# haoxiangsnr/Wave-U-Net-for-Speech-Enhancement

Hardware: AMD Instinct MI355X
Metric: 16384-sample frames/sec fwd+bwd, 12-level Wave-U-Net (higher is better)
Workload: dtype f32 (levels >= 16 samples: 3 x f16 MFMA on hi/lo fp16 halves, fp32 accumulate; the rest f32 MFMA); 1 GPU; unet_basic 12-level, 16384-sample frames, batch=64 per GPU, fp32, training-mode forward + smooth_l1 + backward + fused HIP Adam step (BASELINE.json configs[2]; configs[3] when n_gpus>1); global_batch=64, frame=16384, parallelism=dp1

## Files before the change

wave-u-net-for-speech-enhancement_amd/csrc/wunet_elementwise.h:

```cpp
#pragma once
#include "wunet_dev.h"

struct PackDesc {
    const float* w;
    float* dst;
    int Cout, Cin, taps;
    int M;
    int CP;
    int mtiles;
    int transposed;
};

#define WUNET_MAX_CONV_LAYERS 34
struct PackTable { PackDesc d[WUNET_MAX_CONV_LAYERS]; };

static __global__ __launch_bounds__(WUNET_THREADS) void pack_weights_kernel(PackTable tab)
{
    const PackDesc& d = tab.d[blockIdx.y];
    const int total = d.mtiles * d.CP * d.taps * 16;
    const int kc = d.transposed ? d.Cout : d.Cin;
    for (int idx = blockIdx.x * WUNET_THREADS + threadIdx.x; idx < total; idx += gridDim.x * WUNET_THREADS) {
        const int i = idx & 15;
        int r = idx >> 4;
        const int t = r % d.taps; r /= d.taps;
        const int c = r % d.CP;
        const int mt = r / d.CP;
        const int m = mt * 16 + i;
        float v = 0.0f;
        if (m < d.M && c < kc) {
            v = d.transposed ? d.w[((size_t)c * d.Cin + m) * d.taps + (d.taps - 1 - t)]
                             : d.w[((size_t)m * d.Cin + c) * d.taps + t];
        }
        d.dst[idx] = v;
    }
}

template <int N>
__device__ __forceinline__ void block_sum(double (&a)[N], double* red)
{
// ... 1213 lines not shown
```

wave-u-net-for-speech-enhancement_amd/csrc/wunet_forward.cpp:

```cpp
#include "wunet_host.h"
#include "wunet_elementwise.h"
#include "wunet_tiny.h"
#include "wunet_h3_elem.h"

using namespace wunet_host;

namespace {
struct FwdMode {
    bool training, save;
    const unsigned char* frozen;
    bool is_frozen(int i) const { return frozen && i >= 0 && frozen[i] != 0; }
};

bool skip_handoff(const wunet_ctx* c, int d, const FwdMode& m)
{
    if (!m.training || d <= c->n || d >= c->NL) return false;
    const LayerPlan& dl = c->ly[d];
    return dl.skip_from > 0 && !dl.h3u_train && !m.is_frozen(dl.src0) && !m.is_frozen(dl.src1);
}
bool evop_handoff(const wunet_ctx* c, int p, const FwdMode& m) { return !m.training && p >= 0 && p < c->NL && c->ly[p].evop; }

enum { OP_NONE = 0, OP_IN_CONV, OP_BY_PRODUCER, OP_PREP_H3, OP_SCALAR, OP_DECIM, OP_UPCAT };
enum { CV_FIRST = 0, CV_H3U, CV_H3, CV_TINY, CV_FP32 };
enum { BOUND_NONE = 0, BOUND_EPILOGUE, BOUND_REDUCE, BOUND_ACT_MAX };
// ... 78 lines not shown
};
struct FwdSides { wunet_ctx::Side* fwd = nullptr; wunet_ctx::Side* bwd = nullptr; };

int fork_side(wunet_ctx::Side* side, hipStream_t st)
{
    if (hipEventRecord(side->ev_fork, st) != hipSuccess || hipStreamWaitEvent(side->stream, side->ev_fork, 0) != hipSuccess)
        return fail(WUNET_E_RUNTIME, "fork onto the side stream failed");
    return WUNET_OK;
}

int pack_fp32(const FwdCall& k, hipStream_t pst)
{
    wunet_ctx* c = k.c;
    PackTable tab{};
    int nd = 0;
    for (int i = 0; i < c->NL; ++i) {
        const LayerPlan& l = c->ly[i];
        if (l.h3f || l.first) continue;
        PackDesc& d = tab.d[nd++];
        d.w = k.params[4 * i]; d.dst = k.ws + c->wpkf_off + l.f_wpk;
        d.Cout = l.cout; d.Cin = l.cin; d.taps = l.taps; d.M = l.cout; d.CP = l.f.cp; d.mtiles = l.f.mtiles_p; d.transposed = 0;
    }
    if (nd > 0) {
        WUNET_LAUNCH(pack_weights_kernel, dim3(pack_gx(), nd), dim3(WUNET_THREADS), 0, pst, tab);
        WUNET_CHECK_LAUNCH();
    }
    return WUNET_OK;
}

int pack_split(const FwdCall& k, hipStream_t pst)
{
    wunet_ctx* c = k.c; float* ws = k.ws;
    const bool training = k.m.training;
    {
        ScaleTable T{};
        bool any = false;
        for (int i = 0; i < c->NL; ++i) {
            const LayerPlan& l = c->ly[i];
            ScaleDesc& d = T.d[i];
            d.w = (l.h3f || l.h3d) ? k.params[4 * i] : nullptr; d.wn = (unsigned)((size_t)l.cout * l.cin * l.taps);
            d.gamma = k.params[4 * i + 2]; d.beta = k.params[4 * i + 3]; d.C = l.cout;
            d.sqrtn = sqrtf((float)((double)c->B * l.Lt));
            d.frozen = k.m.is_frozen(i) ? 1 : 0;
            d.zp0 = l.h3f ? ws + l.xzp : nullptr;
            d.zp1 = (l.h3d && training && k.m.save) ? ws + l.gzp : nullptr;
            any = any || l.h3f;
        }
        T.wmax = ws + c->wmax_off; T.slots = x_scale_slot(c, ws, 0); T.training = training ? 1 : 0;
        if (any) {
            WUNET_LAUNCH(h3_scales_kernel, dim3(WUNET_WMAX_PARTS, c->NL), dim3(WUNET_THREADS), 0, pst, T);
            WUNET_CHECK_LAUNCH();
        }
    }
    PackH3Table tab{};
    int nd = 0;
    wunet_half* wh = reinterpret_cast<wunet_half*>(ws + c->h3_wf_hi);
    wunet_half* wl = reinterpret_cast<wunet_half*>(ws + c->h3_wf_lo);
    for (int i = 0; i < c->NL; ++i) {
        const LayerPlan& l = c->ly[i];
        if (!l.h3f) continue;
        PackH3Desc& d = tab.d[nd++];
        d.w = k.params[4 * i]; d.hi = wh + l.h3f_wpk; d.lo = wl + l.h3f_wpk;
        d.Cout = l.cout; d.Cin = l.cin; d.taps = l.taps; d.rows = l.cout; d.kch = l.cin; d.mtiles = l.hf.mtp; d.nch = l.hf.nch; d.transposed = 0;
        d.ntt = (training ? l.h3u_train : l.h3u) ? 0 : l.hf.ntt; d.nfull = ((l.cin + 7) / 8) / 4; d.ns = h3_stage_count(l.cin, l.taps, d.ntt);
        d.wmax = ws + c->wmax_off + (size_t)WUNET_WMAX_PARTS * i; d.wsc = w_scale_slot(c, ws, i);
        d.bf = c->bf;
    }
    if (nd > 0) {
        WUNET_LAUNCH(pack_h3_kernel, dim3(pack_gx(), nd), dim3(WUNET_THREADS), 0, pst, tab);
        WUNET_CHECK_LAUNCH();
    }
    if (!training) {
        RowL1Table rt{};
        int nr = 0;
        for (int i = 0; i < c->NL; ++i) {
            const LayerPlan& l = c->ly[i];
            if (!l.evop) continue;
            RowL1Desc& d = rt.d[nr++];
            d.w = k.params[4 * i]; d.dst = ws + l.wl1; d.rows = l.cout; d.rowlen = l.cin * l.taps;
        }
        if (nr > 0) {
            WUNET_LAUNCH(w_rowl1_kernel, dim3(8, nr), dim3(WUNET_THREADS), 0, pst, rt);
            WUNET_CHECK_LAUNCH();
        }
    }
    return WUNET_OK;
}

int forward_packs(const FwdCall& k, bool packs_valid, void* workspace, FwdSides& sides)
{
    wunet_ctx* c = k.c; float* ws = k.ws; const hipStream_t st = k.st;
    const bool training = k.m.training;
// ... 284 lines not shown
```

wave-u-net-for-speech-enhancement_amd/csrc/wunet_h3_elem.h:

```cpp
#pragma once
#include "wunet_elementwise.h"
#include "wunet_h3.h"

#define WUNET_SLOT_FLOATS 8
#define WUNET_WMAX_PARTS 64
struct ScaleDesc {
    const float* w; unsigned wn;
    const float* gamma; const float* beta; int C;
    float sqrtn;
    int frozen;
    float* zp0; float* zp1;
};
struct ScaleTable { ScaleDesc d[WUNET_MAX_CONV_LAYERS]; float* wmax; float* slots; int training; };

static __global__ __launch_bounds__(WUNET_THREADS) void h3_scales_kernel(ScaleTable T)
{
    __shared__ float red[WUNET_THREADS];
    const ScaleDesc& d = T.d[blockIdx.y];
    const int tid = threadIdx.x;
    if (d.w) {
        float m = 0.0f;
        for (unsigned i = blockIdx.x * WUNET_THREADS + tid; i < d.wn; i += gridDim.x * WUNET_THREADS) m = fmaxf(m, fabsf(d.w[i]));
        red[tid] = m;
        __syncthreads();
        for (int s = WUNET_THREADS / 2; s > 0; s >>= 1) {
            if (tid < s) red[tid] = fmaxf(red[tid], red[tid + s]);
            __syncthreads();
        }
        if (tid == 0) T.wmax[blockIdx.y * WUNET_WMAX_PARTS + blockIdx.x] = red[0];
        __syncthreads();
    }
    if (blockIdx.x == 0) {
        float m = 0.0f;
        if (T.training && !d.frozen)
            for (int c = tid; c < d.C; c += WUNET_THREADS) m = fmaxf(m, fabsf(d.gamma[c]) * d.sqrtn + fabsf(d.beta[c]));
        red[tid] = m;
        __syncthreads();
        for (int s = WUNET_THREADS / 2; s > 0; s >>= 1) {
            if (tid < s) red[tid] = fmaxf(red[tid], red[tid + s]);
            __syncthreads();
        }
        if (tid == 0) T.slots[blockIdx.y * WUNET_SLOT_FLOATS + 4] = red[0];
        if (tid < 4) {
            if (d.zp0) d.zp0[tid] = 0.0f;
            if (d.zp1) d.zp1[tid] = 0.0f;
        }
    }
}

struct RowL1Desc { const float* w; float* dst; int rows, rowlen; };
struct RowL1Table { RowL1Desc d[WUNET_MAX_CONV_LAYERS]; };
static __global__ __launch_bounds__(WUNET_THREADS) void w_rowl1_kernel(RowL1Table T)
{
    __shared__ float red[WUNET_WAVES];
    const RowL1Desc& d = T.d[blockIdx.y];
    for (int r = blockIdx.x; r < d.rows; r += gridDim.x) {
        const float* wr = d.w + (size_t)r * d.rowlen;
        float m = 0.0f;
        for (int i = threadIdx.x; i < d.rowlen; i += WUNET_THREADS) m += fabsf(wr[i]);
#pragma unroll
        for (int k = 1; k < 64; k <<= 1) m += wunet_shfl_xor(m, k);
        __syncthreads();
        if ((threadIdx.x & 63) == 0) red[threadIdx.x >> 6] = m;
        __syncthreads();
        if (threadIdx.x == 0) d.dst[r] = (red[0] + red[1]) + (red[2] + red[3]);
    }
}

static __global__ __launch_bounds__(WUNET_THREADS) void h3_slots_clear_kernel(ScaleTable T, int nl)
{
// ... 440 lines not shown
                    wunet_put_half(l, e, d);
                }
                wunet_sth8(A.sh + (srow * (size_t)(2 * A.L) + (size_t)q) * 8, h);
                if (!A.bf) wunet_sth8(A.sl + (srow * (size_t)(2 * A.L) + (size_t)q) * 8, l);
            }
        }
    }
}

struct PackH3Desc {
    const float* w;
    wunet_half* hi;
    wunet_half* lo;
    int Cout, Cin, taps;
    int rows, kch;
    int mtiles, nch;
    int transposed;
    const float* wmax;
    float* wsc;
    int bf;
    int ntt;
    int nfull, ns;
};
struct PackH3Table { PackH3Desc d[WUNET_MAX_CONV_LAYERS]; };

static __global__ __launch_bounds__(WUNET_THREADS) void pack_h3_kernel(PackH3Table tab)
{
    const PackH3Desc& d = tab.d[blockIdx.y];
    const int ntg = d.taps / 5, ns = d.ntt ? d.ns : d.nch * ntg, nfs = d.ntt ? d.nfull * ntg : ns;
    const int total = d.mtiles * ns * 5 * 512;
    __shared__ float wsc_sh[2];
    if (threadIdx.x < 64) {
        float m = threadIdx.x < WUNET_WMAX_PARTS ? d.wmax[threadIdx.x] : 0.0f;
#pragma unroll
        for (int k = 1; k < 64; k <<= 1) m = fmaxf(m, wunet_shfl_xor(m, k));
        if (threadIdx.x == 0) {
            float s_, i_;
            wunet_pow2_scale(m, s_, i_);
            wsc_sh[0] = s_; wsc_sh[1] = i_;
            if (blockIdx.x == 0 && d.wsc) { d.wsc[0] = s_; d.wsc[1] = i_; }
        }
    }
    __syncthreads();
    const float wscale = wsc_sh[0];
    for (int idx = blockIdx.x * WUNET_THREADS + threadIdx.x; idx < total; idx += gridDim.x * WUNET_THREADS) {
        const int e = idx & 7, i = (idx >> 3) & 15, q = (idx >> 7) & 3;
        int r = idx >> 9;
        const int slot = r % 5; r /= 5;
        const int stg = r % ns, mt = r / ns;
        const int row = mt * 16 + i;
        int k, t;
        if (stg < nfs) { k = (stg / ntg) * 32 + q * 8 + e; t = (stg % ntg) * 5 + slot; }
        else { k = d.nfull * 32 + (stg - nfs) * 8 + e; t = slot < d.ntt ? q * d.ntt + slot : d.taps; }
        float v = 0.0f;
        if (row < d.rows && k < d.kch && t < d.taps)
            v = d.transposed ? d.w[((size_t)k * d.Cin + row) * d.taps + (d.taps - 1 - t)] : d.w[((size_t)row * d.Cin + k) * d.taps + t];
        wunet_half a, b;
        wunet_split_rt(d.bf, wscale * v, a, b);
        d.hi[idx] = a;
        if (!d.bf) d.lo[idx] = b;
    }
}
```

wave-u-net-for-speech-enhancement_amd/csrc/wunet_host.h:

```cpp
#pragma once
#include <cstdarg>
#include <cmath>
#include <cstdio>
#include <cstdlib>
#include <cstring>
#include <map>
#include <mutex>
#include <string>
#include <vector>

#include "wunet_kernels.h"
#include "wunet_h3.h"
#include "wunet_h3u.h"
#include "wunet_launch.h"
#include "wunet_hip.h"

namespace wunet_host {

int fail(int code, const char* fmt, ...);
const char* last_error_text();

#define WUNET_CHECK_LAUNCH()                                                                   \
    do {                                                                                       \
        hipError_t e_ = hipGetLastError();                                                     \
// ... 8 lines not shown

inline int ilog2(long long v) { int r = 0; while ((1LL << r) < v) ++r; return r; }
inline bool is_pow2(long long v) { return v > 0 && (v & (v - 1)) == 0; }
inline size_t align64(size_t v) { return (v + 63) & ~(size_t)63; }
inline int round_up(int v, int m) { return (v + m - 1) / m * m; }
inline unsigned capped_blocks(size_t n, size_t per_block, size_t cap) { const size_t b = (n + per_block - 1) / per_block; return (unsigned)(b < cap ? b : cap); }
inline int kc_of(int taps) { return wunet_lds::conv_mfma(taps, 1).kc; }

struct ConvCfg { int mrep, nrep, mtiles_p, mblocks, cp, grid_x, ksplit, kcps; };
ConvCfg plan_conv(int B, int L, int rows, int kch, int taps);
ConvArgs make_conv_args(const float* x, int kch, const float* wpk, const float* bias, float* out, float* stats,
                        int B, int rows, int L, int taps, const ConvCfg& c, size_t split_stride);
int launch_conv(int taps, const ConvArgs& a, const ConvCfg& c, hipStream_t st);

struct WgradCfg { int mrep, nw, xit, wsplit, mblocks, nblocks, ksplit, cps, rows; };
WgradCfg plan_wgrad(int B, int L, int cin, int cout, int taps);
WgradArgs make_wgrad_args(const float* x, const float* g, float* part, int B, int Cin, int Cout, int L, int taps, int cps);
int launch_wgrad_any(int taps, const WgradArgs& a, const WgradCfg& w, hipStream_t st);

enum { LK_RAW = 0, LK_DECIM = 1, LK_UPCAT = 2 };

struct PlanSwitches {
    const char *order_f, *order_d, *order_w;
    bool no_split, old_split, ktail_off, no_skip_fuse, no_evop, no_e0, no_enc_gz, pa_swap_off, upt_off, wgrad_xcd_off;
    int sps, h3u_eval, h3u_train, a_cap;
};
PlanSwitches read_plan_switches();

struct H3ConvPlan { int mrep, mtp, nch, sps, ksplit, ntiles, ntt; };
H3ConvPlan plan_h3_conv(int B, int L, int rows, int kch, int taps, bool transposed, int bf, const PlanSwitches& sw);
struct H3WgradPlan { int mrep, mblocks, nblocks, ksplit, cps, tp, xcd, dma, db; };
H3WgradPlan plan_h3_wgrad(int B, int L, int cin, int cout, int taps, int bf, const PlanSwitches& sw);

struct LayerGeom {
    int cin, cout, taps, L, logL, kind;
    int Lt;
    int src0, src1;
    int c0;
};
struct LayerDecisions {
    ConvCfg f;
    ConvCfg d;
    WgradCfg w;
    int f_rows;
    int a_split;
    size_t f_wpk, d_wpk;
    size_t z, a, s, mean, rstd, xin, g, dx, k1, k2, k3;
// ... 16 lines not shown
struct LayerPlan : LayerGeom, LayerDecisions {};

int h3_stage_count(int kch, int taps, int ntt);
size_t h3w_part_stride(const LayerGeom& g, const H3WgradPlan& w);
int wgrad_blocks_per_cu(const WgradCfg& w, int L, int taps);
int h3w_blocks_per_cu(int taps, int mrep, int L);
bool up_pairs_regular(int Lin);
unsigned pack_gx();

}

struct wunet_ctx {
    int n, ci, B, T, NL;
    int Tt = 0;
    bool padded = false;
    size_t pad_in = 0, pad_out = 0, pad_gout = 0;
    std::vector<wunet_host::LayerPlan> ly;
    size_t stats_off, wpkf_off, spart_off, fwd_floats;
    size_t bmax_off, bound_off;
    size_t bpart_off, wgpart_off, wpkb_off, gh_off, hpart_off, hpart2_off, e0part_off, total_floats;
    int e0 = 1;
    int enc_gz = 1;
    int pa_swap = 1;
    int head_blocks;
    int h3 = 0;
    int bf = 0;
    std::vector<unsigned char> frozen;
    bool any_frozen = false;
    size_t h3_wf_hi, h3_wf_lo, h3_wb_hi, h3_wb_lo, h3_slot;
    size_t fslot_off, wmax_off;
    size_t h3_wf_halfs, h3_wb_halfs;
    struct Side {
        hipStream_t stream = nullptr; hipEvent_t ev_fork = nullptr, ev_join = nullptr, ev_pack = nullptr, ev_fpack = nullptr, ev_fpack2 = nullptr;
        const void* packed_ws = nullptr;
    };
    std::map<int, Side> side;
    std::mutex side_lock;
};

namespace wunet_host {

void layout_workspace(wunet_ctx* c);
int launch_split(const float* x, wunet_half* hi, wunet_half* lo, const float* sc, const float* xb0, const float* xb1, float* xsc,
                 int B, int C, int L, hipStream_t st, int bf = 0);
float* x_scale_slot(const wunet_ctx* c, float* ws, int layer);
float* w_scale_slot(const wunet_ctx* c, float* ws, int layer);
// ... 25 lines not shown
```

wave-u-net-for-speech-enhancement_amd/csrc/wunet_launchers.cpp:

```cpp
#include "wunet_host.h"
#include "wunet_elementwise.h"
#include "wunet_h3_elem.h"

namespace wunet_host {

static int lds_refused(const char* kernel, size_t smem)
{
    return fail(WUNET_E_ARG, "%s: %zu bytes of dynamic LDS requested, its layout needs %zu", kernel, smem, wunet_lds_needed);
}

ConvArgs make_conv_args(const float* x, int kch, const float* wpk, const float* bias, float* out, float* stats,
                        int B, int rows, int L, int taps, const ConvCfg& c, size_t split_stride)
{
    ConvArgs a{};
    a.x = x; a.wpk = wpk; a.bias = bias; a.out = out; a.stats = stats;
    a.B = B; a.Cin = kch; a.Cout = rows; a.CinP = c.cp; a.L = L; a.logL = ilog2(L);
    const int tn = 64 * c.nrep;
    a.seg = L < tn ? L : tn;
    a.seg_shift = ilog2(a.seg);
    a.segw = a.seg + 16;
    const int rowlen = wunet_lds::staged_row(L, tn);
    a.rowp = wunet_lds::conv_mfma_rowp(L, c.nrep);
    a.r4 = rowlen / 4;
    a.sw4 = a.segw / 4;
// ... 184 lines not shown
        WgradH3Args a{};
        fill(a);
        rc = wunet_launch_wgrad_h3(a, l.taps, w.mrep, nseg, tp, grid, smem, st, bf != 0);
    }
    prof_end(st);
    if (rc == WUNET_LAUNCH_E_LDS) return lds_refused(pname, smem);
    if (rc != 0) return fail(WUNET_E_ARG, "no wgrad_h3 kernel for taps=%d mrep=%d (rc %d)", l.taps, w.mrep, rc);
    return 0;
}

int launch_backward_packs(wunet_ctx* c, const float* const* params, float* ws, hipStream_t st)
{
    const int NL = c->NL;
    PackTable tab{};
    int nd = 0;
    for (int i = 1; i < NL; ++i) {
        const LayerPlan& l = c->ly[i];
        if (l.h3d) continue;
        PackDesc& d = tab.d[nd++];
        d.w = params[4 * i]; d.dst = ws + c->wpkb_off + l.d_wpk;
        d.Cout = l.cout; d.Cin = l.cin; d.taps = l.taps; d.M = l.cin; d.CP = l.d.cp; d.mtiles = l.d.mtiles_p; d.transposed = 1;
    }
    if (nd > 0) {
        WUNET_LAUNCH(pack_weights_kernel, dim3(pack_gx(), nd), dim3(WUNET_THREADS), 0, st, tab);
        WUNET_CHECK_LAUNCH();
    }
    if (c->h3) {
        PackH3Table t3{};
        int n3 = 0;
        wunet_half* wh = reinterpret_cast<wunet_half*>(ws + c->h3_wb_hi);
        wunet_half* wl = reinterpret_cast<wunet_half*>(ws + c->h3_wb_lo);
        for (int i = 1; i < NL; ++i) {
            const LayerPlan& l = c->ly[i];
            if (!l.h3d) continue;
            PackH3Desc& d = t3.d[n3++];
            d.w = params[4 * i]; d.hi = wh + l.h3d_wpk; d.lo = wl + l.h3d_wpk;
            d.Cout = l.cout; d.Cin = l.cin; d.taps = l.taps; d.rows = l.cin; d.kch = l.cout; d.mtiles = l.hd.mtp; d.nch = l.hd.nch; d.transposed = 1;
            d.ntt = l.hd.ntt; d.nfull = ((l.cout + 7) / 8) / 4; d.ns = h3_stage_count(l.cout, l.taps, l.hd.ntt);
            d.wmax = ws + c->wmax_off + (size_t)WUNET_WMAX_PARTS * i;
            d.wsc = l.h3f ? nullptr : w_scale_slot(c, ws, i);
            d.bf = c->bf;
        }
        if (n3 > 0) {
            WUNET_LAUNCH(pack_h3_kernel, dim3(pack_gx(), n3), dim3(WUNET_THREADS), 0, st, t3);
            WUNET_CHECK_LAUNCH();
        }
    }
    return 0;
}

bool side_stream_off()
{
    static const bool off = getenv("WUNET_NO_SIDE_STREAM") != nullptr;
    return off;
}

wunet_ctx::Side* side_for_current_device(wunet_ctx* c)
{
    int dev = 0;
    if (hipGetDevice(&dev) != hipSuccess) { fail(WUNET_E_RUNTIME, "hipGetDevice failed"); return nullptr; }
    std::lock_guard<std::mutex> g(c->side_lock);
    auto it = c->side.find(dev);
    if (it != c->side.end()) return &it->second;
    wunet_ctx::Side sd;
    const unsigned evf = hipEventDisableTiming | (unsigned)hipEventDisableSystemFence;
    if (hipStreamCreateWithFlags(&sd.stream, hipStreamNonBlocking) != hipSuccess ||
        hipEventCreateWithFlags(&sd.ev_fork, evf) != hipSuccess ||
// ... 12 lines not shown
```

wave-u-net-for-speech-enhancement_amd/csrc/wunet_ops.cpp:

```cpp
#include "wunet_host.h"
#include "wunet_elementwise.h"
#include "wunet_h3_elem.h"
#include "wunet_loss_rows.h"
#include "wunet_stft.h"
#include "wunet_stoi.h"
#include "wunet_estoi.h"
#include "wunet_mix.h"
#include "wunet_reverb.h"

using namespace wunet_host;

extern "C" {

size_t wunet_loss_scratch_bytes(void) { return 256 * sizeof(double); }

int wunet_loss_forward(int kind, const float* clean, const float* enhanced, size_t n, float* loss_out, void* scratch, void* stream)
{
    if (kind < 0 || kind > 2 || !clean || !enhanced || !loss_out || !scratch || n == 0) return fail(WUNET_E_ARG, "bad loss argument");
    hipStream_t st = (hipStream_t)stream;
    const unsigned blocks = capped_blocks(n, WUNET_THREADS * 8, 256);
    WUNET_LAUNCH(loss_partial_kernel, dim3(blocks), dim3(WUNET_THREADS), 0, st, kind, clean, enhanced, n, (double*)scratch);
    WUNET_CHECK_LAUNCH();
    WUNET_LAUNCH(loss_final_kernel, dim3(1), dim3(WUNET_THREADS), 0, st, (const double*)scratch, (int)blocks, n, loss_out);
    WUNET_CHECK_LAUNCH();
// ... 744 lines not shown
    prof_end(st);
    WUNET_CHECK_LAUNCH();
    return WUNET_OK;
}

static int op_check(int B, int Cin, int Cout, int L, int K)
{
    if (K != 5 && K != 15) return fail(WUNET_E_ARG, "K must be 5 or 15");
    if (B < 1 || Cin < 1 || Cout < 1 || !is_pow2(L) || L < 4) return fail(WUNET_E_ARG, "bad op shape (L must be a power of two >= 4)");
    return 0;
}

static int op_conv_common(const float* x, const float* w, const float* bias, float* out, int B, int kch, int rows,
                          int Cout, int Cin, int L, int K, int transposed, hipStream_t st)
{
    const ConvCfg cfg = plan_conv(B, L, rows, kch, K);
    float *wpk = nullptr, *part = nullptr;
    if (hipMalloc((void**)&wpk, (size_t)cfg.mtiles_p * cfg.cp * K * 16 * sizeof(float)) != hipSuccess) return fail(WUNET_E_RUNTIME, "hipMalloc");
    const size_t nout = (size_t)B * rows * L;
    if (cfg.ksplit > 1 && hipMalloc((void**)&part, (size_t)cfg.ksplit * nout * sizeof(float)) != hipSuccess) return fail(WUNET_E_RUNTIME, "hipMalloc");
    PackTable tab{};
    PackDesc& d = tab.d[0];
    d.w = w; d.dst = wpk; d.Cout = Cout; d.Cin = Cin; d.taps = K; d.M = rows; d.CP = cfg.cp; d.mtiles = cfg.mtiles_p; d.transposed = transposed;
    WUNET_LAUNCH(pack_weights_kernel, dim3(64, 1), dim3(WUNET_THREADS), 0, st, tab);
    const bool split = cfg.ksplit > 1;
    const ConvArgs a = make_conv_args(x, kch, wpk, split ? nullptr : bias, split ? part : out, nullptr, B, rows, L, K, cfg, nout);
    int rc = launch_conv(K, a, cfg, st);
    if (!rc && split) {
        WUNET_LAUNCH(split_sum_kernel, dim3(capped_blocks(nout, WUNET_THREADS, 2048)), dim3(WUNET_THREADS), 0, st, (const float*)part, cfg.ksplit, nout, out,
                     bias, rows, ilog2(L));
    }
    hipStreamSynchronize(st);
    hipFree(wpk);
    if (part) hipFree(part);
    if (rc) return rc;
    WUNET_CHECK_LAUNCH();
    return WUNET_OK;
}

int wunet_op_conv1d(const float* x, const float* w, const float* bias, float* z, int B, int Cin, int Cout, int L, int K, void* stream)
{
    if (op_check(B, Cin, Cout, L, K)) return WUNET_E_ARG;
    return op_conv_common(x, w, bias, z, B, Cin, Cout, Cout, Cin, L, K, 0, (hipStream_t)stream);
}

int wunet_op_conv1d_dgrad(const float* gz, const float* w, float* dx, int B, int Cin, int Cout, int L, int K, void* stream)
{
// ... 60 lines not shown
}

int op_conv_split_common(const float* x, const float* w, const float* bias, float* out, int B, int kch, int rows, int Cout, int Cin,
                         int L, int K, int transposed, int bf, hipStream_t st)
{
    const H3ConvPlan p = plan_h3_conv(B, L, rows, kch, K, transposed != 0, bf, read_plan_switches());
    SplitBuf xs;
    DevBuf wpk, misc, part;
    const size_t wh_halfs = (size_t)p.mtp * p.nch * K * 512, nout = (size_t)B * rows * L;
    if (!wpk.alloc(wh_halfs * 4) || !misc.alloc((16 + WUNET_WMAX_PARTS + 2 * (size_t)kch) * sizeof(float)) ||
        (p.ksplit > 1 && !part.alloc((size_t)p.ksplit * nout * sizeof(float))))
        return fail(WUNET_E_RUNTIME, "hipMalloc");
    float* xslot = misc.f(), *wslot = misc.f() + 8, *wmax = misc.f() + 16, *oz = misc.f() + 16 + WUNET_WMAX_PARTS;
    WUNET_LAUNCH(fill_kernel, dim3(4), dim3(WUNET_THREADS), 0, st, oz, (size_t)kch, 1.0f);
    WUNET_LAUNCH(fill_kernel, dim3(4), dim3(WUNET_THREADS), 0, st, oz + kch, (size_t)kch, 0.0f);
    wunet_half* const whp = wpk.h();
    wunet_half* const wlp = wpk.h() + wh_halfs;
    int rc = op_split_operand(x, B, kch, L, xs, xslot, oz, oz + kch, bf, st);
    if (rc) return rc;
    {
        ScaleTable T{};
        T.d[0].w = w; T.d[0].wn = (unsigned)((size_t)Cout * Cin * K); T.d[0].gamma = oz; T.d[0].beta = oz; T.d[0].C = 1; T.d[0].sqrtn = 0.0f;
        T.wmax = wmax; T.slots = wslot; T.training = 0;
        WUNET_LAUNCH(h3_scales_kernel, dim3(WUNET_WMAX_PARTS, 1), dim3(WUNET_THREADS), 0, st, T);
        PackH3Table tab{};
        PackH3Desc& d = tab.d[0];
        d.w = w; d.hi = whp; d.lo = wlp; d.Cout = Cout; d.Cin = Cin; d.taps = K; d.rows = rows; d.kch = kch; d.mtiles = p.mtp; d.nch = p.nch;
        d.ntt = p.ntt; d.nfull = ((kch + 7) / 8) / 4; d.ns = h3_stage_count(kch, K, p.ntt);
        d.transposed = transposed; d.wmax = wmax; d.wsc = wslot + 2; d.bf = bf;
        WUNET_LAUNCH(pack_h3_kernel, dim3(64, 1), dim3(WUNET_THREADS), 0, st, tab);
    }
    const bool split = p.ksplit > 1;
    ConvH3Launch h{};
    h.taps = K; h.mrep = p.mrep; h.mtiles_p = p.mtp; h.sps = p.sps; h.nch = p.nch; h.ntt = p.ntt;
    h.B = B; h.rows = rows; h.kch = kch; h.L = L; h.bf = bf;
    h.xh = xs.h(); h.xl = xs.l(); h.zpad = xs.zpad(); h.wh = whp; h.wl = wlp;
    h.bias = split ? nullptr : bias; h.sc = xslot; h.sc2 = wslot + 2; h.out = split ? part.f() : out;
    rc = launch_conv_h3(h, st);
    if (!rc && split) {
        const unsigned blocks = capped_blocks(nout, WUNET_THREADS, 2048);
        const float* partp = part.f();
        const int ks = p.ksplit;
        char pname[48];
        snprintf(pname, sizeof pname, "split_sum_kernel<%d>", ks);
        prof_begin(st, pname, 0.0, 4.0 * (ks + 1.0) * nout);
        WUNET_LAUNCH(split_sum_kernel, dim3(blocks), dim3(WUNET_THREADS), 0, st, partp, ks, nout, out, bias, rows, ilog2(L));
        prof_end(st);
    }
    hipStreamSynchronize(st);
    if (rc) return rc;
    WUNET_CHECK_LAUNCH();
    return WUNET_OK;
}
// ... 69 lines not shown
```

wave-u-net-for-speech-enhancement_amd/csrc/wunet_plan.cpp:

```cpp
#include <algorithm>
#include "wunet_host.h"
#include "wunet_h3_elem.h"

namespace wunet_host {

namespace { thread_local std::string g_err; }

int fail(int code, const char* fmt, ...)
{
    char buf[512];
    va_list ap;
    va_start(ap, fmt);
    vsnprintf(buf, sizeof buf, fmt, ap);
    va_end(ap);
    g_err = buf;
    return code;
}

const char* last_error_text() { return g_err.c_str(); }

namespace {
struct ProfRec { std::string name; double flops; double bytes; hipEvent_t e0, e1; };
std::vector<ProfRec> g_prof;
}
// ... 163 lines not shown
    w.rows = w.ksplit * (w.wsplit ? 4 : 1);
    return w;
}
unsigned pack_gx() { return 512; }

PlanSwitches read_plan_switches()
{
    const auto is_zero = [](const char* name) { const char* e = getenv(name); return e != nullptr && atoi(e) == 0; };
    PlanSwitches sw{};
    sw.order_f = getenv("WUNET_H3_ORDER"); sw.order_d = getenv("WUNET_H3D_ORDER"); sw.order_w = getenv("WUNET_H3W_ORDER");
    sw.no_split = getenv("WUNET_H3_NOSPLIT") != nullptr; sw.old_split = getenv("WUNET_H3_OLDSPLIT") != nullptr;
    if (const char* e = getenv("WUNET_H3_SPS")) sw.sps = atoi(e);
    sw.ktail_off = is_zero("WUNET_H3_KTAIL");
    sw.h3u_eval = 512; sw.h3u_train = 2048;
    if (const char* e = getenv("WUNET_H3U")) {
        int a = 0, b = 0;
        const int got = sscanf(e, "%d,%d", &a, &b);
        if (got == 2) { sw.h3u_eval = a; sw.h3u_train = b; }
        else if (got == 1) sw.h3u_eval = sw.h3u_train = a;
    }
    sw.no_skip_fuse = getenv("WUNET_NO_SKIP_FUSE") != nullptr; sw.no_evop = getenv("WUNET_NO_EVOP") != nullptr; sw.no_e0 = getenv("WUNET_NO_E0") != nullptr;
    sw.no_enc_gz = getenv("WUNET_NO_ENC_GZ") != nullptr; sw.pa_swap_off = is_zero("WUNET_PA_SWAP");
    sw.upt_off = is_zero("WUNET_UPT"); sw.wgrad_xcd_off = is_zero("WUNET_WGRAD_XCD");
    sw.a_cap = getenv("WUNET_A_CAP") ? atoi(getenv("WUNET_A_CAP")) : 128;
    return sw;
}

int pick_mrep_h3(int mtiles, const char* ord)
{
    int best = 2, best_pad = 1 << 30;
    for (const char* p = ord; *p; ++p) {
        const int m = *p - '0';
        const int pad = round_up(mtiles, m) - mtiles;
        if (pad < best_pad) { best_pad = pad; best = m; }
    }
    return best;
}

const char* h3_order(int taps, int L, int ntiles, int mtiles)
{
    return (taps == 5 && L >= 256 && (long long)ntiles * ((mtiles + 3) / 4) >= 512) ? "432" : "32";
}

size_t h3w_part_stride(const LayerGeom& g, const H3WgradPlan& w)
{
    const int tw = g.taps == 15 ? 8 : 5;
// ... 131 lines not shown
        l.h3x = l.h3w;
        if (l.h3f) {
            l.hf = plan_h3_conv(B, l.L, l.cout, l.cin, l.taps, false, c->bf, sw);
            l.f.ksplit = l.hf.ksplit;
            l.f.grid_x = l.hf.ntiles;
        }
        if (l.h3d) {
            l.hd = plan_h3_conv(B, l.L, l.cin, l.cout, l.taps, true, c->bf, sw);
            l.d.ksplit = l.hd.ksplit;
        }
        if (l.h3w) l.hw = plan_h3_wgrad(B, l.L, l.cin, l.cout, l.taps, c->bf, sw);
        if (l.first) { l.f.ksplit = 1; l.f.grid_x = (int)(((long long)B * l.L + 1023) / 1024); }
        const bool can = h3u_can_run(c, l);
        l.h3u = (can && sw.h3u_eval > 0 && l.L >= sw.h3u_eval) ? 1 : 0;
        l.h3u_train = (can && sw.h3u_train > 0 && l.L >= sw.h3u_train) ? 1 : 0;
        l.f_rows = l.h3f ? l.f.grid_x : l.f.grid_x * WUNET_WAVES;
        const long long sp = posn / 4096;
        const int a_cap = sw.a_cap < 1 ? 1 : (sw.a_cap > 256 ? 256 : sw.a_cap);
        l.a_split = (int)(sp < 1 ? 1 : (sp > a_cap ? a_cap : sp));
    }
    const long long hb = ((long long)B * c->T) / 2048;
    c->head_blocks = (int)(hb < 1 ? 1 : (hb > 1024 ? 1024 : hb));
    c->e0 = sw.no_e0 ? 0 : 1;
    c->enc_gz = sw.no_enc_gz ? 0 : 1;
    c->pa_swap = sw.pa_swap_off ? 0 : 1;
}

static bool skip_planned(const LayerPlan& e, const LayerPlan& d) { return e.kind == LK_DECIM && d.kind == LK_UPCAT && e.h3x && d.h3x && d.src1 == e.src0 && d.c0 % 8 == 0; }
static bool evop_planned(const wunet_ctx* c, const LayerPlan& p, const LayerPlan& q, int pi)
{
    return p.h3f && !p.first && p.taps == 15 && p.L >= 256 && p.f.ksplit == 1 && p.hf.mrep <= 4 && q.kind == LK_DECIM && q.src0 == pi && q.h3f && q.h3x &&
           !c->bf && !c->padded;
}
static bool upt_planned(const wunet_ctx* c, const LayerPlan& q, const LayerPlan& p)
{
    return q.kind == LK_UPCAT && q.h3d && q.L >= 256 && q.d.ksplit == 1 && !(q.c0 & 3) && !(q.cin & 3) && q.c0 == p.cout && !c->bf && !c->padded &&
           p.h3d && p.L >= 128 && up_pairs_regular(q.L / 2);
}
static void plan_handoffs(wunet_ctx* c, const PlanSwitches& sw)
{
    for (int i = 1; i <= c->n && !sw.no_skip_fuse; ++i) {
        LayerPlan& d = c->ly[2 * c->n - i + 1];
        if (skip_planned(c->ly[i], d)) d.skip_from = i;
    }
    for (int i = 1; i + 1 <= c->n && !sw.no_evop; ++i)
        if (evop_planned(c, c->ly[i], c->ly[i + 1], i)) c->ly[i].evop = 1;
// ... 204 lines not shown
```

Before: 12770 frames/s.

## Pack weights through LDS tiles with coalesced vector loads instead of strided gathers

Replaces the per-element gather weight packing kernels (fp32 and hi/lo fp16 split) with tiled kernels. Each block loads a 16-row by 32-channel weight tile into shared memory using aligned float4 loads, then writes packed output with vector stores, and the grid is flattened across layers through a prefix table. The weight abs-max scale kernel is also vectorised with float4 loads and wave shuffles. The old gather kernels remain available behind WUNET_PACK_GATHER. Weight packing runs every step, so this targets the per-step pre-processing cost, at the expense of more complex code and handling for misalignment and tails.

```diff
diff --git a/wave-u-net-for-speech-enhancement_amd/csrc/wunet_elementwise.h b/wave-u-net-for-speech-enhancement_amd/csrc/wunet_elementwise.h
--- a/wave-u-net-for-speech-enhancement_amd/csrc/wunet_elementwise.h
+++ b/wave-u-net-for-speech-enhancement_amd/csrc/wunet_elementwise.h
@@ -12,9 +12,119 @@
 };
 
 #define WUNET_MAX_CONV_LAYERS 34
-struct PackTable { PackDesc d[WUNET_MAX_CONV_LAYERS]; };
-
+struct PackTable { PackDesc d[WUNET_MAX_CONV_LAYERS]; int first[WUNET_MAX_CONV_LAYERS + 1]; };
+
+template <int TAPS, bool TR, int PAD>
+struct WTileShape {
+    static constexpr int RUNS = TR ? 32 : 16, LEN = (TR ? 16 : 32) * TAPS, STRIDE = LEN + PAD;
+    static constexpr int NPR = LEN / 4 + 1;
+    static constexpr int PPL = (NPR + 63) / 64;
+    static constexpr int NLD = RUNS / WUNET_WAVES * PPL;
+    static __device__ __forceinline__ int at(int i, int kk, int t) { return TR ? kk * STRIDE + i * TAPS + (TAPS - 1 - t) : i * STRIDE + kk * TAPS + t; }
+};
+#define WUNET_WTILE_FLOATS (32 * (16 * 15 + 2))
+struct WTileSrc { unsigned start, step; int nruns, nlen; };
+__device__ __forceinline__ int wunet_clampi(int v, int hi) { return v < 0 ? 0 : (v > hi ? hi : v); }
+__device__ __forceinline__ WTileSrc wunet_wtile_src(bool transposed, int Cin, int taps, int row0, int nrows, int k0, int nk)
+{
+    WTileSrc T;
+    T.step = (unsigned)(Cin * taps);
+    if (transposed) { T.start = ((unsigned)k0 * Cin + row0) * taps; T.nruns = nk; T.nlen = nrows * taps; }
+    else { T.start = ((unsigned)row0 * Cin + k0) * taps; T.nruns = nrows; T.nlen = nk * taps; }
+    return T;
+}
+template <class S>
+__device__ __forceinline__ void wunet_wtile_load(float* tile, const float* w, const WTileSrc& T)
+{
+    float ev = 0.0f;
+    int eat = -1;
+    {
+        const int r = (int)threadIdx.x >> 3, k = (int)threadIdx.x & 7;
+        if (r < T.nruns) {
+            const float* a = w + (T.start + (unsigned)r * T.step);
+            const int mis = (int)(((size_t)a >> 2) & 3), g = k < 4 ? 0 : (T.nlen + mis) / 4, p = 4 * g - mis, pos = p + (k & 3);
+            const bool whole = p >= 0 && p + 4 <= T.nlen;
+            if ((k < 4 || g > 0) && !whole && pos >= 0 && pos < T.nlen) { ev = a[pos]; eat = r * S::STRIDE + pos; }
+        }
+    }
+    const int wave = wunet_uniform((int)threadIdx.x >> 6), lane = (int)threadIdx.x & 63;
+    wunet_f4 v[S::NLD];
+    bool ld[S::NLD];
+#pragma unroll
+    for (int k = 0; k < S::NLD; ++k) {
+        const int r = wave + WUNET_WAVES * (k / S::PPL), g = lane + 64 * (k % S::PPL);
+        ld[k] = false;
+        if (r < T.nruns && g < S::NPR) {
+            const float* a = w + (T.start + (unsigned)r * T.step);
+            const int p = 4 * g - (int)(((size_t)a >> 2) & 3);
+            if (p >= 0 && p + 4 <= T.nlen) { v[k] = wunet_ld4(a + p); ld[k] = true; }
+        }
+    }
+    if (eat >= 0) tile[eat] = ev;
+#pragma unroll
+    for (int k = 0; k < S::NLD; ++k) {
+        const int r = wave + WUNET_WAVES * (k / S::PPL), g = lane + 64 * (k % S::PPL);
+        if (g >= S::NPR) continue;
+        const bool in = r < T.nruns;
+        const int mis = in ? (int)(((size_t)(w + (T.start + (unsigned)r * T.step)) >> 2) & 3) : 0, p = 4 * g - mis;
+        if (ld[k]) {
+#pragma unroll
+            for (int e = 0; e < 4; ++e) tile[r * S::STRIDE + p + e] = v[k][e];
+        } else {
+            const int ne = in ? T.nlen : 0;
+#pragma unroll
+            for (int e = 0; e < 4; ++e) {
+                const int q = p + e;
+                if (q >= ne && q < S::LEN) tile[r * S::STRIDE + q] = 0.0f;
+            }
+        }
+    }
+}
+
+template <int TAPS, bool TR>
+__device__ __forceinline__ void pack_weights_tile(const PackDesc& d, int mt, int ch, float* tile)
+{
+    typedef WTileShape<TAPS, TR, 2> S;
+    const int kc = TR ? d.Cout : d.Cin;
+    wunet_wtile_load<S>(tile, d.w, wunet_wtile_src(TR, d.Cin, TAPS, mt * 16, wunet_clampi(d.M - mt * 16, 16), ch * 32, wunet_clampi(kc - ch * 32, 32)));
+    __syncthreads();
+    const int np = wunet_clampi(d.CP - ch * 32, 32) * TAPS * 4;
+    float* out = d.dst + ((size_t)mt * d.CP + ch * 32) * TAPS * 16;
+    for (int p = threadIdx.x; p < np; p += WUNET_THREADS) {
+        const int i4 = p & 3, ct = p >> 2, cc = ct / TAPS, t = ct - cc * TAPS;
+        wunet_f4 v;
+#pragma unroll
+        for (int j = 0; j < 4; ++j) v[j] = tile[S::at(i4 * 4 + j, cc, t)];
+        wunet_st4(out + 4 * (size_t)p, v);
+    }
+}
 static __global__ __launch_bounds__(WUNET_THREADS) void pack_weights_kernel(PackTable tab)
+{
+    __shared__ float tile[WUNET_WTILE_FLOATS];
+    int li = 0;
+    while ((int)blockIdx.x >= tab.first[li + 1]) ++li;
+    const PackDesc& d = tab.d[li];
+    const int nch = (d.CP + 31) / 32, u = (int)blockIdx.x - tab.first[li], mt = u / nch, ch = u - mt * nch;
+    if (d.taps == 15) {
+        if (d.transposed) pack_weights_tile<15, true>(d, mt, ch, tile);
+        else pack_weights_tile<15, false>(d, mt, ch, tile);
+    } else {
+        if (d.transposed) pack_weights_tile<5, true>(d, mt, ch, tile);
+        else pack_weights_tile<5, false>(d, mt, ch, tile);
+    }
+}
+
+inline unsigned pack_table_blocks(PackTable& tab, int nd)
+{
+    int n = 0;
+    for (int i = 0; i <= WUNET_MAX_CONV_LAYERS; ++i) {
+        tab.first[i] = n;
+        if (i < nd) n += tab.d[i].mtiles * ((tab.d[i].CP + 31) / 32);
+    }
+    return (unsigned)n;
+}
+
+static __global__ __launch_bounds__(WUNET_THREADS) void pack_weights_gather_kernel(PackTable tab)
 {
     const PackDesc& d = tab.d[blockIdx.y];
     const int total = d.mtiles * d.CP * d.taps * 16;
diff --git a/wave-u-net-for-speech-enhancement_amd/csrc/wunet_forward.cpp b/wave-u-net-for-speech-enhancement_amd/csrc/wunet_forward.cpp
--- a/wave-u-net-for-speech-enhancement_amd/csrc/wunet_forward.cpp
+++ b/wave-u-net-for-speech-enhancement_amd/csrc/wunet_forward.cpp
@@ -124,7 +124,9 @@
         d.Cout = l.cout; d.Cin = l.cin; d.taps = l.taps; d.M = l.cout; d.CP = l.f.cp; d.mtiles = l.f.mtiles_p; d.transposed = 0;
     }
     if (nd > 0) {
-        WUNET_LAUNCH(pack_weights_kernel, dim3(pack_gx(), nd), dim3(WUNET_THREADS), 0, pst, tab);
+        const unsigned tiles = pack_table_blocks(tab, nd);
+        if (c->pack_gather) WUNET_LAUNCH(pack_weights_gather_kernel, dim3(pack_gx(), nd), dim3(WUNET_THREADS), 0, pst, tab);
+        else WUNET_LAUNCH(pack_weights_kernel, dim3(tiles), dim3(WUNET_THREADS), 0, pst, tab);
         WUNET_CHECK_LAUNCH();
     }
     return WUNET_OK;
@@ -150,7 +152,8 @@
         }
         T.wmax = ws + c->wmax_off; T.slots = x_scale_slot(c, ws, 0); T.training = training ? 1 : 0;
         if (any) {
-            WUNET_LAUNCH(h3_scales_kernel, dim3(WUNET_WMAX_PARTS, c->NL), dim3(WUNET_THREADS), 0, pst, T);
+            if (c->pack_gather) WUNET_LAUNCH(h3_scales_gather_kernel, dim3(WUNET_WMAX_PARTS, c->NL), dim3(WUNET_THREADS), 0, pst, T);
+            else WUNET_LAUNCH(h3_scales_kernel, dim3(WUNET_WMAX_PARTS, c->NL), dim3(WUNET_THREADS), 0, pst, T);
             WUNET_CHECK_LAUNCH();
         }
     }
@@ -169,7 +172,9 @@
         d.bf = c->bf;
     }
     if (nd > 0) {
-        WUNET_LAUNCH(pack_h3_kernel, dim3(pack_gx(), nd), dim3(WUNET_THREADS), 0, pst, tab);
+        const unsigned tiles = pack_table_blocks(tab, nd);
+        if (c->pack_gather) WUNET_LAUNCH(pack_h3_gather_kernel, dim3(pack_gx(), nd), dim3(WUNET_THREADS), 0, pst, tab);
+        else WUNET_LAUNCH(pack_h3_kernel, dim3(tiles), dim3(WUNET_THREADS), 0, pst, tab);
         WUNET_CHECK_LAUNCH();
     }
     if (!training) {
diff --git a/wave-u-net-for-speech-enhancement_amd/csrc/wunet_h3_elem.h b/wave-u-net-for-speech-enhancement_amd/csrc/wunet_h3_elem.h
--- a/wave-u-net-for-speech-enhancement_amd/csrc/wunet_h3_elem.h
+++ b/wave-u-net-for-speech-enhancement_amd/csrc/wunet_h3_elem.h
@@ -13,7 +13,72 @@
 };
 struct ScaleTable { ScaleDesc d[WUNET_MAX_CONV_LAYERS]; float* wmax; float* slots; int training; };
 
+__device__ __forceinline__ void h3_scales_bound(const ScaleTable& T, const ScaleDesc& d, float* red)
+{
+    const int tid = threadIdx.x;
+    {
+        float m = 0.0f;
+        if (T.training && !d.frozen)
+            for (int c = tid; c < d.C; c += WUNET_THREADS) m = fmaxf(m, fabsf(d.gamma[c]) * d.sqrtn + fabsf(d.beta[c]));
+        red[tid] = m;
+        __syncthreads();
+        for (int s = WUNET_THREADS / 2; s > 0; s >>= 1) {
+            if (tid < s) red[tid] = fmaxf(red[tid], red[tid + s]);
+            __syncthreads();
+        }
+        if (tid == 0) T.slots[blockIdx.y * WUNET_SLOT_FLOATS + 4] = red[0];
+        if (tid < 4) {
+            if (d.zp0) d.zp0[tid] = 0.0f;
+            if (d.zp1) d.zp1[tid] = 0.0f;
+        }
+    }
+}
+
+__device__ __forceinline__ float wunet_absmax4(float m, wunet_f4 v)
+{
+    return fmaxf(fmaxf(m, fabsf(v[0])), fmaxf(fmaxf(fabsf(v[1]), fabsf(v[2])), fabsf(v[3])));
+}
+
 static __global__ __launch_bounds__(WUNET_THREADS) void h3_scales_kernel(ScaleTable T)
+{
+    __shared__ float red[WUNET_THREADS];
+    const ScaleDesc& d = T.d[blockIdx.y];
+    const int tid = threadIdx.x;
+    if (d.w) {
+        const unsigned mis = (unsigned)(((size_t)d.w >> 2) & 3), h4 = (4u - mis) & 3u, head = h4 < d.wn ? h4 : d.wn;
+        const unsigned n4 = (d.wn - head) / 4, tail = d.wn - head - 4 * n4, stride = gridDim.x * WUNET_THREADS;
+        const float* body = d.w + head;
+        float m0 = 0.0f, m1 = 0.0f, m2 = 0.0f, m3 = 0.0f;
+        unsigned i = blockIdx.x * WUNET_THREADS + tid;
+        for (; i + 7 * stride < n4; i += 8 * stride) {
+            wunet_f4 v[8];
+#pragma unroll
+            for (int k = 0; k < 8; ++k) v[k] = wunet_ld4(body + 4 * (size_t)(i + k * stride));
+            m0 = wunet_absmax4(wunet_absmax4(m0, v[0]), v[4]); m1 = wunet_absmax4(wunet_absmax4(m1, v[1]), v[5]);
+            m2 = wunet_absmax4(wunet_absmax4(m2, v[2]), v[6]); m3 = wunet_absmax4(wunet_absmax4(m3, v[3]), v[7]);
+        }
+        for (; i + 3 * stride < n4; i += 4 * stride) {
+            const wunet_f4 v0 = wunet_ld4(body + 4 * (size_t)i), v1 = wunet_ld4(body + 4 * (size_t)(i + stride));
+            const wunet_f4 v2 = wunet_ld4(body + 4 * (size_t)(i + 2 * stride)), v3 = wunet_ld4(body + 4 * (size_t)(i + 3 * stride));
+            m0 = wunet_absmax4(m0, v0); m1 = wunet_absmax4(m1, v1); m2 = wunet_absmax4(m2, v2); m3 = wunet_absmax4(m3, v3);
+        }
+        for (; i < n4; i += stride) m0 = wunet_absmax4(m0, wunet_ld4(body + 4 * (size_t)i));
+        if (blockIdx.x == 0) {
+            if ((unsigned)tid < head) m1 = fmaxf(m1, fabsf(d.w[tid]));
+            if ((unsigned)tid < tail) m2 = fmaxf(m2, fabsf(body[4 * (size_t)n4 + tid]));
+        }
+        float m = fmaxf(fmaxf(m0, m1), fmaxf(m2, m3));
+#pragma unroll
+        for (int k = 1; k < 64; k <<= 1) m = fmaxf(m, wunet_shfl_xor(m, k));
+        if ((tid & 63) == 0) red[tid >> 6] = m;
+        __syncthreads();
+        if (tid == 0) T.wmax[blockIdx.y * WUNET_WMAX_PARTS + blockIdx.x] = fmaxf(fmaxf(red[0], red[1]), fmaxf(red[2], red[3]));
+        __syncthreads();
+    }
+    if (blockIdx.x == 0) h3_scales_bound(T, d, red);
+}
+
+static __global__ __launch_bounds__(WUNET_THREADS) void h3_scales_gather_kernel(ScaleTable T)
 {
     __shared__ float red[WUNET_THREADS];
     const ScaleDesc& d = T.d[blockIdx.y];
@@ -30,22 +95,7 @@
         if (tid == 0) T.wmax[blockIdx.y * WUNET_WMAX_PARTS + blockIdx.x] = red[0];
         __syncthreads();
     }
-    if (blockIdx.x == 0) {
-        float m = 0.0f;
-        if (T.training && !d.frozen)
-            for (int c = tid; c < d.C; c += WUNET_THREADS) m = fmaxf(m, fabsf(d.gamma[c]) * d.sqrtn + fabsf(d.beta[c]));
-        red[tid] = m;
-        __syncthreads();
-        for (int s = WUNET_THREADS / 2; s > 0; s >>= 1) {
-            if (tid < s) red[tid] = fmaxf(red[tid], red[tid + s]);
-            __syncthreads();
-        }
-        if (tid == 0) T.slots[blockIdx.y * WUNET_SLOT_FLOATS + 4] = red[0];
-        if (tid < 4) {
-            if (d.zp0) d.zp0[tid] = 0.0f;
-            if (d.zp1) d.zp1[tid] = 0.0f;
-        }
-    }
+    if (blockIdx.x == 0) h3_scales_bound(T, d, red);
 }
 
 struct RowL1Desc { const float* w; float* dst; int rows, rowlen; };
@@ -532,25 +582,104 @@
     int ntt;
     int nfull, ns;
 };
-struct PackH3Table { PackH3Desc d[WUNET_MAX_CONV_LAYERS]; };
-
-static __global__ __launch_bounds__(WUNET_THREADS) void pack_h3_kernel(PackH3Table tab)
-{
-    const PackH3Desc& d = tab.d[blockIdx.y];
-    const int ntg = d.taps / 5, ns = d.ntt ? d.ns : d.nch * ntg, nfs = d.ntt ? d.nfull * ntg : ns;
-    const int total = d.mtiles * ns * 5 * 512;
-    __shared__ float wsc_sh[2];
+struct PackH3Table { PackH3Desc d[WUNET_MAX_CONV_LAYERS]; int first[WUNET_MAX_CONV_LAYERS + 1]; };
+
+__device__ __forceinline__ float pack_h3_wmax(const PackH3Desc& d)
+{
+    return threadIdx.x < WUNET_WMAX_PARTS ? d.wmax[threadIdx.x] : 0.0f;
+}
+__device__ __forceinline__ void pack_h3_scale(const PackH3Desc& d, float m, float* wsc_sh, bool publish)
+{
     if (threadIdx.x < 64) {
-        float m = threadIdx.x < WUNET_WMAX_PARTS ? d.wmax[threadIdx.x] : 0.0f;
 #pragma unroll
         for (int k = 1; k < 64; k <<= 1) m = fmaxf(m, wunet_shfl_xor(m, k));
         if (threadIdx.x == 0) {
             float s_, i_;
             wunet_pow2_scale(m, s_, i_);
             wsc_sh[0] = s_; wsc_sh[1] = i_;
-            if (blockIdx.x == 0 && d.wsc) { d.wsc[0] = s_; d.wsc[1] = i_; }
-        }
-    }
+            if (publish && d.wsc) { d.wsc[0] = s_; d.wsc[1] = i_; }
+        }
+    }
+}
+__host__ __device__ inline int pack_h3_chunks(const PackH3Desc& d)
+{
+    return d.ntt ? d.nfull + (d.ns > d.nfull * (d.taps / 5) ? 1 : 0) : d.nch;
+}
+
+template <int TAPS, bool TR>
+__device__ __forceinline__ void pack_h3_tile(const PackH3Desc& d, int mt, int ch, bool publish, float* tile, float* wsc_sh)
+{
+    typedef WTileShape<TAPS, TR, 1> S;
+    constexpr int ntg = TAPS / 5;
+    const int ns = d.ntt ? d.ns : d.nch * ntg, nfs = d.ntt ? d.nfull * ntg : ns;
+    const float wm = pack_h3_wmax(d);
+    wunet_wtile_load<S>(tile, d.w, wunet_wtile_src(TR, d.Cin, TAPS, mt * 16, wunet_clampi(d.rows - mt * 16, 16), ch * 32, wunet_clampi(d.kch - ch * 32, 32)));
+    pack_h3_scale(d, wm, wsc_sh, publish);
+    __syncthreads();
+    const float wscale = wsc_sh[0];
+    const bool tail = ch * ntg >= nfs;
+    const int stg0 = tail ? nfs : ch * ntg, np = (tail ? ns - nfs : ntg) * 5 * 64;
+    const size_t base = ((size_t)mt * ns + stg0) * (5 * 512);
+    const auto pieces = [&](auto bf) {
+        constexpr bool BF = decltype(bf)::value;
+        for (int p = threadIdx.x; p < np; p += WUNET_THREADS) {
+            const int i = p & 15, q = (p >> 4) & 3, ss = p >> 6, sg = ss / 5, slot = ss - sg * 5;
+            const int kk = tail ? sg * 8 : q * 8;
+            int t = tail ? (slot < d.ntt ? q * d.ntt + slot : TAPS) : sg * 5 + slot;
+            const bool has = t < TAPS;
+            t = has ? t : 0;
+            const float* src = tile + S::at(i, kk, t);
+            wunet_h8 h, l;
+#pragma unroll
+            for (int e = 0; e < 8; ++e) {
+                wunet_half a, b;
+                float x = src[S::at(0, e, 0) - S::at(0, 0, 0)];
+                x = has ? x : 0.0f;
+                wunet_split<BF>(wscale * x, a, b);
+                wunet_put_half(h, e, a);
+                wunet_put_half(l, e, b);
+            }
+            wunet_sth8(d.hi + base + 8 * (size_t)p, h);
+            if (!BF) wunet_sth8(d.lo + base + 8 * (size_t)p, l);
+        }
+    };
+    if (d.bf) pieces(std::true_type{});
+    else pieces(std::false_type{});
+}
+static __global__ __launch_bounds__(WUNET_THREADS) void pack_h3_kernel(PackH3Table tab)
+{
+    __shared__ float tile[WUNET_WTILE_FLOATS];
+    __shared__ float wsc_sh[2];
+    int li = 0;
+    while ((int)blockIdx.x >= tab.first[li + 1]) ++li;
+    const PackH3Desc& d = tab.d[li];
+    const int nu = pack_h3_chunks(d), u = (int)blockIdx.x - tab.first[li], mt = u / nu, ch = u - mt * nu;
+    if (d.taps == 15) {
+        if (d.transposed) pack_h3_tile<15, true>(d, mt, ch, u == 0, tile, wsc_sh);
+        else pack_h3_tile<15, false>(d, mt, ch, u == 0, tile, wsc_sh);
+    } else {
+        if (d.transposed) pack_h3_tile<5, true>(d, mt, ch, u == 0, tile, wsc_sh);
+        else pack_h3_tile<5, false>(d, mt, ch, u == 0, tile, wsc_sh);
+    }
+}
+
+inline unsigned pack_table_blocks(PackH3Table& tab, int nd)
+{
+    int n = 0;
+    for (int i = 0; i <= WUNET_MAX_CONV_LAYERS; ++i) {
+        tab.first[i] = n;
+        if (i < nd) n += tab.d[i].mtiles * pack_h3_chunks(tab.d[i]);
+    }
+    return (unsigned)n;
+}
+
+static __global__ __launch_bounds__(WUNET_THREADS) void pack_h3_gather_kernel(PackH3Table tab)
+{
+    const PackH3Desc& d = tab.d[blockIdx.y];
+    const int ntg = d.taps / 5, ns = d.ntt ? d.ns : d.nch * ntg, nfs = d.ntt ? d.nfull * ntg : ns;
+    const int total = d.mtiles * ns * 5 * 512;
+    __shared__ float wsc_sh[2];
+    pack_h3_scale(d, pack_h3_wmax(d), wsc_sh, blockIdx.x == 0);
     __syncthreads();
     const float wscale = wsc_sh[0];
     for (int idx = blockIdx.x * WUNET_THREADS + threadIdx.x; idx < total; idx += gridDim.x * WUNET_THREADS) {
diff --git a/wave-u-net-for-speech-enhancement_amd/csrc/wunet_host.h b/wave-u-net-for-speech-enhancement_amd/csrc/wunet_host.h
--- a/wave-u-net-for-speech-enhancement_amd/csrc/wunet_host.h
+++ b/wave-u-net-for-speech-enhancement_amd/csrc/wunet_host.h
@@ -54,7 +54,7 @@
 
 struct PlanSwitches {
     const char *order_f, *order_d, *order_w;
-    bool no_split, old_split, ktail_off, no_skip_fuse, no_evop, no_e0, no_enc_gz, pa_swap_off, upt_off, wgrad_xcd_off;
+    bool no_split, old_split, ktail_off, no_skip_fuse, no_evop, no_e0, no_enc_gz, pa_swap_off, upt_off, wgrad_xcd_off, pack_gather;
     int sps, h3u_eval, h3u_train, a_cap;
 };
 PlanSwitches read_plan_switches();
@@ -117,6 +117,7 @@
     int e0 = 1;
     int enc_gz = 1;
     int pa_swap = 1;
+    int pack_gather = 0;
     int head_blocks;
     int h3 = 0;
     int bf = 0;
diff --git a/wave-u-net-for-speech-enhancement_amd/csrc/wunet_launchers.cpp b/wave-u-net-for-speech-enhancement_amd/csrc/wunet_launchers.cpp
--- a/wave-u-net-for-speech-enhancement_amd/csrc/wunet_launchers.cpp
+++ b/wave-u-net-for-speech-enhancement_amd/csrc/wunet_launchers.cpp
@@ -230,7 +230,9 @@
         d.Cout = l.cout; d.Cin = l.cin; d.taps = l.taps; d.M = l.cin; d.CP = l.d.cp; d.mtiles = l.d.mtiles_p; d.transposed = 1;
     }
     if (nd > 0) {
-        WUNET_LAUNCH(pack_weights_kernel, dim3(pack_gx(), nd), dim3(WUNET_THREADS), 0, st, tab);
+        const unsigned tiles = pack_table_blocks(tab, nd);
+        if (c->pack_gather) WUNET_LAUNCH(pack_weights_gather_kernel, dim3(pack_gx(), nd), dim3(WUNET_THREADS), 0, st, tab);
+        else WUNET_LAUNCH(pack_weights_kernel, dim3(tiles), dim3(WUNET_THREADS), 0, st, tab);
         WUNET_CHECK_LAUNCH();
     }
     if (c->h3) {
@@ -250,7 +252,9 @@
             d.bf = c->bf;
         }
         if (n3 > 0) {
-            WUNET_LAUNCH(pack_h3_kernel, dim3(pack_gx(), n3), dim3(WUNET_THREADS), 0, st, t3);
+            const unsigned tiles = pack_table_blocks(t3, n3);
+            if (c->pack_gather) WUNET_LAUNCH(pack_h3_gather_kernel, dim3(pack_gx(), n3), dim3(WUNET_THREADS), 0, st, t3);
+            else WUNET_LAUNCH(pack_h3_kernel, dim3(tiles), dim3(WUNET_THREADS), 0, st, t3);
             WUNET_CHECK_LAUNCH();
         }
     }
diff --git a/wave-u-net-for-speech-enhancement_amd/csrc/wunet_ops.cpp b/wave-u-net-for-speech-enhancement_amd/csrc/wunet_ops.cpp
--- a/wave-u-net-for-speech-enhancement_amd/csrc/wunet_ops.cpp
+++ b/wave-u-net-for-speech-enhancement_amd/csrc/wunet_ops.cpp
@@ -790,7 +790,9 @@
     PackTable tab{};
     PackDesc& d = tab.d[0];
     d.w = w; d.dst = wpk; d.Cout = Cout; d.Cin = Cin; d.taps = K; d.M = rows; d.CP = cfg.cp; d.mtiles = cfg.mtiles_p; d.transposed = transposed;
-    WUNET_LAUNCH(pack_weights_kernel, dim3(64, 1), dim3(WUNET_THREADS), 0, st, tab);
+    const unsigned tiles = pack_table_blocks(tab, 1);
+    if (read_plan_switches().pack_gather) WUNET_LAUNCH(pack_weights_gather_kernel, dim3(64, 1), dim3(WUNET_THREADS), 0, st, tab);
+    else WUNET_LAUNCH(pack_weights_kernel, dim3(tiles), dim3(WUNET_THREADS), 0, st, tab);
     const bool split = cfg.ksplit > 1;
     const ConvArgs a = make_conv_args(x, kch, wpk, split ? nullptr : bias, split ? part : out, nullptr, B, rows, L, K, cfg, nout);
     int rc = launch_conv(K, a, cfg, st);
@@ -897,13 +899,17 @@
         ScaleTable T{};
         T.d[0].w = w; T.d[0].wn = (unsigned)((size_t)Cout * Cin * K); T.d[0].gamma = oz; T.d[0].beta = oz; T.d[0].C = 1; T.d[0].sqrtn = 0.0f;
         T.wmax = wmax; T.slots = wslot; T.training = 0;
-        WUNET_LAUNCH(h3_scales_kernel, dim3(WUNET_WMAX_PARTS, 1), dim3(WUNET_THREADS), 0, st, T);
+        const bool gather = read_plan_switches().pack_gather;
+        if (gather) WUNET_LAUNCH(h3_scales_gather_kernel, dim3(WUNET_WMAX_PARTS, 1), dim3(WUNET_THREADS), 0, st, T);
+        else WUNET_LAUNCH(h3_scales_kernel, dim3(WUNET_WMAX_PARTS, 1), dim3(WUNET_THREADS), 0, st, T);
         PackH3Table tab{};
         PackH3Desc& d = tab.d[0];
         d.w = w; d.hi = whp; d.lo = wlp; d.Cout = Cout; d.Cin = Cin; d.taps = K; d.rows = rows; d.kch = kch; d.mtiles = p.mtp; d.nch = p.nch;
         d.ntt = p.ntt; d.nfull = ((kch + 7) / 8) / 4; d.ns = h3_stage_count(kch, K, p.ntt);
         d.transposed = transposed; d.wmax = wmax; d.wsc = wslot + 2; d.bf = bf;
-        WUNET_LAUNCH(pack_h3_kernel, dim3(64, 1), dim3(WUNET_THREADS), 0, st, tab);
+        const unsigned tiles = pack_table_blocks(tab, 1);
+        if (gather) WUNET_LAUNCH(pack_h3_gather_kernel, dim3(64, 1), dim3(WUNET_THREADS), 0, st, tab);
+        else WUNET_LAUNCH(pack_h3_kernel, dim3(tiles), dim3(WUNET_THREADS), 0, st, tab);
     }
     const bool split = p.ksplit > 1;
     ConvH3Launch h{};
diff --git a/wave-u-net-for-speech-enhancement_amd/csrc/wunet_plan.cpp b/wave-u-net-for-speech-enhancement_amd/csrc/wunet_plan.cpp
--- a/wave-u-net-for-speech-enhancement_amd/csrc/wunet_plan.cpp
+++ b/wave-u-net-for-speech-enhancement_amd/csrc/wunet_plan.cpp
@@ -209,6 +209,7 @@
     sw.no_skip_fuse = getenv("WUNET_NO_SKIP_FUSE") != nullptr; sw.no_evop = getenv("WUNET_NO_EVOP") != nullptr; sw.no_e0 = getenv("WUNET_NO_E0") != nullptr;
     sw.no_enc_gz = getenv("WUNET_NO_ENC_GZ") != nullptr; sw.pa_swap_off = is_zero("WUNET_PA_SWAP");
     sw.upt_off = is_zero("WUNET_UPT"); sw.wgrad_xcd_off = is_zero("WUNET_WGRAD_XCD");
+    { const char* e = getenv("WUNET_PACK_GATHER"); sw.pack_gather = e != nullptr && atoi(e) != 0; }
     sw.a_cap = getenv("WUNET_A_CAP") ? atoi(getenv("WUNET_A_CAP")) : 128;
     return sw;
 }
@@ -386,6 +387,7 @@
     const long long hb = ((long long)B * c->T) / 2048;
     c->head_blocks = (int)(hb < 1 ? 1 : (hb > 1024 ? 1024 : hb));
     c->e0 = sw.no_e0 ? 0 : 1;
+    c->pack_gather = sw.pack_gather ? 1 : 0;
     c->enc_gz = sw.no_enc_gz ? 0 : 1;
     c->pa_swap = sw.pa_swap_off ? 0 : 1;
 }
```

Result: no change. 12800 frames/s (median of 6 runs) (+0.3%).
